# jibanCat/gp_dla_detection

Measured on AMD Instinct MI355X. Metric: sample log-likelihoods/sec (n~1500,k=20), higher is better.
Workload: dtype f64; 1 GPU; BASELINE configs[1]: synthetic spectra, fused Voigt + low-rank log-evidence sweep, HBM-resident; spectra_per_gpu=1000, pixels=1500, k=20, dla_samples=10000, num_lines=3, parallelism=spectra sharded over 1 GPU(s), RCCL all-gather of the 15-column posterior table

## Files before the change

### gp_dla_detection_amd/_lib.py

```python
from __future__ import annotations

import ctypes as C
import os
import subprocess

_HERE = os.path.dirname(os.path.abspath(__file__))
CSRC = os.path.join(_HERE, "csrc")
DEFAULT_LIB_PATH = os.path.join(CSRC, "libgpdla.so")


def lib_path() -> str:
    return os.environ.get("GPDLA_LIB_PATH") or DEFAULT_LIB_PATH

HIPCC_FLAGS = ["--offload-arch=gfx950", "-O3", "-ffp-contract=off", "-fPIC", "-shared",
               "-std=c++17", "-no-hip-rt", "-Wno-inline-asm"]

LEGACY_LIB_PATH = os.path.join(CSRC, "libgpdla_legacy.so")

_dp = C.POINTER(C.c_double)
_i64p = C.POINTER(C.c_int64)
_i32p = C.POINTER(C.c_int32)
_u8p = C.POINTER(C.c_uint8)
_u32p = C.POINTER(C.c_uint32)
_f32p = C.POINTER(C.c_float)
# ... 251 lines not shown
    ("gpdla_model_spectra_validate", C.c_int, [C.POINTER(ModelSpectraRequest), C.c_int64, C.c_int64, C.c_int]),
    ("gpdla_batch_unmasked_counts", C.c_int, [C.c_void_p, C.c_void_p, _i64p]),
    ("gpdla_batch_model_spectra", C.c_int, [C.c_void_p, C.c_void_p, C.POINTER(ModelSpectraRequest),
                                            C.POINTER(ModelSpectra)]),
    ("gpdla_model_spectra_multi_validate", C.c_int, [C.POINTER(ModelSpectraMultiRequest), C.c_int64, C.c_int64, C.c_int,
                                                     C.c_int, C.c_int]),
    ("gpdla_batch_model_spectra_multi", C.c_int, [C.c_void_p, C.c_void_p, C.POINTER(ModelSpectraMultiRequest),
                                                  C.POINTER(ModelSpectraMulti)]),
    ("gpdla_debug_profiles_ms", C.c_int, [C.c_void_p, C.c_void_p, _dp]),
    ("gpdla_model_mean", C.c_int, [C.POINTER(Model), C.c_int64, _dp, _i64p, _dp, _dp, C.c_int, C.c_int, C.c_int,
                                   C.c_double, C.c_double, _dp, C.c_int]),
    ("gpdla_mock_validate", C.c_int, [C.POINTER(MockRequest), C.c_int64]),
    ("gpdla_batch_draw_mocks", C.c_int, [C.c_void_p, C.c_void_p, C.POINTER(MockRequest), C.POINTER(MockSpectra)]),
    ("gpdla_samples_kde", C.c_int, [C.c_int64, _dp, C.c_int64, _dp, C.c_double, _dp, _dp, C.c_int]),
    ("gpdla_samples_fit_prior", C.c_int, [C.c_int64, _dp, C.c_double, C.c_double, C.c_double, C.c_double, C.c_double,
                                          C.c_double, C.c_double, C.c_double, C.POINTER(NhiPrior), C.c_int]),
    ("gpdla_samples_prior_eval", C.c_int, [C.POINTER(NhiPrior), C.c_int64, _dp, _dp, _dp, C.c_int]),
    ("gpdla_samples_halton", C.c_int, [C.c_int64, C.c_int64, C.c_int, _i32p, _dp, C.c_int]),
    ("gpdla_samples_draw", C.c_int, [C.POINTER(NhiPrior), C.c_int64, C.c_int64, _dp, C.c_int, C.c_double, C.c_double,
                                     C.POINTER(SampleDraw), C.c_int]),
    ("gpdla_preload_spectra", C.c_int, [C.c_int64, _i64p, _f32p, _f32p, _f32p, _i32p, _dp, _u8p, C.POINTER(PreloadConfig),
                                        _i64p, _dp, _dp, _dp, _u8p, _dp, C.c_int]),
    ("gpdla_stats_parameter_summaries", C.c_int, [C.c_int64, C.c_int64, _dp, C.c_int64, _u32p, _dp, _dp, _dp, _dp,
                                                  C.POINTER(SummaryRequest), C.POINTER(ParameterSummaries), C.c_int]),
    ("gpdla_batch_parameter_summaries", C.c_int, [C.c_void_p, C.c_void_p, C.c_int, C.c_int, _i64p, C.c_int64,
                                                  C.POINTER(SummaryRequest), C.POINTER(ParameterSummaries)]),
    ("gpdla_debug_last_summaries_ms", C.c_double, []),
    ("gpdla_refine_validate", C.c_int, [C.POINTER(RefineRequest), C.POINTER(NhiPrior), C.c_int64, _dp, _dp]),
    ("gpdla_context_set_refine_points", C.c_int, [C.c_void_p, C.c_int64, _dp, _dp]),
    ("gpdla_batch_refine", C.c_int, [C.c_void_p, C.c_void_p, _i64p, C.c_int64, C.POINTER(RefineRequest),
                                     C.POINTER(NhiPrior)]),
    ("gpdla_batch_download_refined", C.c_int, [C.c_void_p, C.c_void_p, _i64p, C.c_int64, C.POINTER(RefinedResults)]),
    ("gpdla_batch_refined_summaries", C.c_int, [C.c_void_p, C.c_void_p, _i64p, C.c_int64, C.POINTER(SummaryRequest),
                                                C.POINTER(ParameterSummaries)]),
    ("gpdla_batch_refined_posteriors", C.c_int, [C.c_void_p, C.c_void_p, _i64p, C.c_int64, C.POINTER(RefinedPosteriors)]),
    ("gpdla_debug_last_refine_ms", C.c_double, []),
    ("gpdla_fixed_absorbers_validate", C.c_int, [C.c_int64, _i64p, _dp, _dp, C.c_double]),
    ("gpdla_batch_set_fixed_absorbers", C.c_int, [C.c_void_p, C.c_void_p, _i64p, _dp, _dp, C.c_double, C.c_int32]),
    ("gpdla_batch_clear_fixed_absorbers", C.c_int, [C.c_void_p, C.c_void_p]),
    ("gpdla_debug_conditioned_rows", C.c_int, [C.c_void_p, C.c_void_p, C.c_int32, C.c_int64, _dp, _dp, C.c_int64, _i64p]),
    ("gpdla_stats_posterior_maps", C.c_int, [C.c_int64, C.c_int64, _dp, C.c_int64, _u32p, _dp, _dp, _dp, _dp, _dp, _dp, _dp, _dp,
                                             _dp, C.POINTER(PosteriorMapsRequest), C.POINTER(PosteriorMaps), C.c_int]),
    ("gpdla_batch_posterior_maps", C.c_int, [C.c_void_p, C.c_void_p, C.c_int, C.c_int, _i64p, C.c_int64, _dp, _dp, _dp, _dp,
                                             _dp, C.POINTER(PosteriorMapsRequest), C.POINTER(PosteriorMaps)]),
    ("gpdla_batch_refined_posterior_maps", C.c_int, [C.c_void_p, C.c_void_p, _i64p, C.c_int64, _dp, _dp, _dp, _dp, _dp,
                                                     C.POINTER(PosteriorMapsRequest), C.POINTER(PosteriorMaps)]),
    ("gpdla_posterior_maps_rows_per_launch", C.c_int64, [C.c_int, C.c_int, C.c_int]),
    ("gpdla_debug_last_maps_ms", C.c_double, [C.c_int]),
    ("gpdla_debug_last_maps_launches", C.c_int64, []),
    ("gpdla_debug_near_poly", C.c_int, [C.c_int, C.c_double, _dp, _dp]),
    ("gpdla_debug_prepared_rows", C.c_int, [C.c_void_p, C.c_void_p, C.c_int, C.c_int64, _dp, C.c_int64, _i64p]),
    ("gpdla_debug_philox4x32_10", None, [_u32p, _u32p, _u32p]),
    ("gpdla_debug_throw", C.c_int, [C.c_int]),
]

_lib = None


def host_sources() -> list:
    import re
    unit = os.path.join(CSRC, "gpdla.hip")
    with open(unit) as f:
        names = re.findall(r'^#include "(host_\w+\.hpp)"', f.read(), flags=re.M)
    return [unit] + [os.path.join(CSRC, n) for n in names]


def _build(out: str, extra_flags, force: bool, verbose: bool) -> str:
    import glob
    srcs = (host_sources() + glob.glob(os.path.join(CSRC, "*.hip")) + glob.glob(os.path.join(CSRC, "*.hpp"))
            + glob.glob(os.path.join(_HERE, "..", "include", "*.h")))
    if not force and os.path.exists(out):
        if all(os.path.getmtime(out) >= os.path.getmtime(s) for s in srcs):
            return out
    cmd = ["hipcc", *HIPCC_FLAGS, *extra_flags, os.path.join(CSRC, "gpdla.hip"), "-o", out]
    res = subprocess.run(cmd, capture_output=True, text=True)
    if verbose or res.returncode:
        print(res.stdout, res.stderr)
    if res.returncode:
        raise RuntimeError(f"hipcc failed building {os.path.basename(out)}:\n" + res.stderr)
    return out


def build(force: bool = False, verbose: bool = False) -> str:
    return _build(DEFAULT_LIB_PATH, [], force, verbose)


def build_legacy(force: bool = False, verbose: bool = False) -> str:
    return _build(LEGACY_LIB_PATH, ["-DGPDLA_WITH_LEGACY"], force, verbose)


def _preload_hip_runtime():
    candidates = []
    try:
        import torch
        candidates.append(os.path.join(os.path.dirname(torch.__file__), "lib", "libamdhip64.so"))
    except Exception:
        pass
    candidates += ["/opt/rocm/lib/libamdhip64.so", "libamdhip64.so"]
    last = None
    for path in candidates:
        if os.path.isabs(path) and not os.path.exists(path):
            continue
        try:
            return C.CDLL(path, mode=C.RTLD_GLOBAL)
        except OSError as e:
            last = e
# ... 26 lines not shown
```

### gp_dla_detection_amd/csrc/host_refine.hpp

```cpp
#pragma once

static_assert(GPDLA_REFINE_MAX_LEVELS == gpdla::kRefineMaxLevels, "gpdla.h and sweep_kernels.hpp disagree");

namespace {

thread_local double t_refine_ms = -1.0;

int validate_refine_request(const gpdla_refine_request *rq, const gpdla_nhi_prior *prior) {
  if (!rq) return fail(GPDLA_ERR_INVALID_ARGUMENT, "null refine request");
  if (rq->levels < 1 || rq->levels > GPDLA_REFINE_MAX_LEVELS)
    return fail(GPDLA_ERR_INVALID_ARGUMENT, "levels = %d outside [1, %d]", rq->levels, GPDLA_REFINE_MAX_LEVELS);
  if (!(rq->delta > 0.0) || !std::isfinite(rq->delta)) return fail(GPDLA_ERR_INVALID_ARGUMENT, "delta = %g must be finite and > 0", rq->delta);
  if (!(rq->pad >= 0.0) || !std::isfinite(rq->pad)) return fail(GPDLA_ERR_INVALID_ARGUMENT, "pad = %g must be finite and >= 0", rq->pad);
  return prior ? check_prior(prior) : GPDLA_OK;
}

int validate_refine_points(int64_t n, const double *u, const double *v) {
  if (n < 1 || n > (1LL << 30)) return fail(GPDLA_ERR_INVALID_ARGUMENT, "num_points = %lld outside [1, 2^30]", (long long)n);
  if (!u || !v) return fail(GPDLA_ERR_INVALID_ARGUMENT, "null u / v");
  for (int64_t j = 0; j < n; ++j) {
    if (!(u[j] >= 0.0 && u[j] < 1.0)) return fail(GPDLA_ERR_INVALID_ARGUMENT, "u[%lld] = %g is not inside [0, 1)", (long long)j, u[j]);
    if (!(v[j] >= 0.0 && v[j] < 1.0)) return fail(GPDLA_ERR_INVALID_ARGUMENT, "v[%lld] = %g is not inside [0, 1)", (long long)j, v[j]);
  }
  return GPDLA_OK;
}

size_t refine_layout(RefineBuffers *rf, char *base, size_t nq, size_t Sr) {
  size_t at = 0;
  auto take = [&](auto *&p, size_t count) {
    using T = std::remove_reference_t<decltype(*p)>;
    if (base) p = reinterpret_cast<T *>(base + at);
    at += (std::max<size_t>(count * sizeof(T), 8) + 255) & ~(size_t)255;
  };
  take(rf->box, nq * kRefineBoxStride);
  take(rf->rmeta, nq);
  take(rf->ell, nq * Sr);
  take(rf->lam, nq * Sr);
  take(rf->ll_scratch, nq);
  take(rf->terms, nq * kRefineTerms * 2);
  take(rf->scal, nq * kRefineScalars);
  take(rf->status, nq);
  take(rf->rows, nq);
  return at;
}

int refine_reserve(gpdla_batch *b, int64_t Sr) {
  if (!b->rf) b->rf = new RefineBuffers();
  RefineBuffers *rf = b->rf;
  if (!rf->ev_rows) HIP_TRY(hipEventCreateWithFlags(&rf->ev_rows, hipEventDisableTiming));
  const size_t need = refine_layout(rf, nullptr, (size_t)b->nq, (size_t)Sr);
  if (!rf->arena || rf->cap_bytes < need) {
    dev_free(rf->arena);
    rf->arena = nullptr;
    rf->cap_bytes = 0;
    void *p = nullptr;
    if (hipMalloc(&p, need) != hipSuccess) return fail(GPDLA_ERR_HIP, "hipMalloc of %zu bytes for the refine tables failed", need);
    rf->arena = p;
    rf->cap_bytes = need;
  }
  refine_layout(rf, static_cast<char *>(rf->arena), (size_t)b->nq, (size_t)Sr);
  rf->nq = b->nq;
  rf->Sr = Sr;
  return GPDLA_OK;
}

int launch_boxed_sweep(gpdla_context *c, gpdla_batch *b, RecordClass cls, int64_t count, const BoxedSweepArgs &args) {
  const bool three = args.num_lines == 3;
  if (cls == kRecSlim20)
    return launch_sweep_kernel(c, three ? &k_sweep_slim_boxed<3> : &k_sweep_slim_boxed<0>, kSweepWaves * 64,
                               (size_t)kSlimLdsDoubles * sizeof(double), kSweepWaves * kSamplesPerWave, count, args);
  const size_t lds = std::max(sweep_split_slim_lds_doubles(false), kExpTab + kSplitEpilogueDoubles) * sizeof(double);
  if (lds > 160 * 1024) return fail(GPDLA_ERR_UNSUPPORTED, "split sweep needs %zu B of LDS", lds);
  return launch_sweep_kernel(c, three ? &k_sweep_split_slim<3, 0, BoxedSweepArgs> : &k_sweep_split_slim<0, 0, BoxedSweepArgs>, 512, lds,
                             2 * kSamplesPerWave, count, args);
}

int check_refinable(gpdla_context *c, gpdla_batch *b) {
  int rc = check_batch_pair(c, b);
  if (rc) return rc;
  if (b->md) return fail(GPDLA_ERR_UNSUPPORTED, "the refine pass serves single-DLA batches only");
  if (c->cfg.contraction_precision == 1) return fail(GPDLA_ERR_UNSUPPORTED, "the refine pass is fp64 only (contraction_precision = 1)");
  if (b->k > 40) return fail(GPDLA_ERR_UNSUPPORTED, "k = %d: the refine pass serves k <= 40", b->k);
  return GPDLA_OK;
}

}

extern "C" {

int gpdla_refine_validate(const gpdla_refine_request *request, const gpdla_nhi_prior *prior, int64_t num_points,
                          const double *u, const double *v) try {
  int rc = validate_refine_request(request, prior);
  if (rc) return rc;
  return (num_points || u || v) ? validate_refine_points(num_points, u, v) : GPDLA_OK;
} GPDLA_NO_THROW

int gpdla_context_set_refine_points(gpdla_context *c, int64_t num_points, const double *u, const double *v) try {
  if (!c) return fail(GPDLA_ERR_INVALID_ARGUMENT, "null context");
  int rc = validate_refine_points(num_points, u, v);
  if (rc) return rc;
  HIP_TRY(hipSetDevice(c->device_id));
  HIP_TRY(hipStreamSynchronize(c->stream));
  dev_free(c->d_ru);
  dev_free(c->d_rv);
  dev_free(c->d_rperm);
  c->d_ru = c->d_rv = nullptr;
  c->d_rperm = nullptr;
  c->Sr = 0;
  const size_t n = (size_t)num_points;
  std::vector<int32_t> perm(n);
  std::iota(perm.begin(), perm.end(), 0);
  std::stable_sort(perm.begin(), perm.end(), [&](int32_t x, int32_t y) { return u[x] < u[y]; });
  if ((rc = upload(&c->d_ru, u, n, c->stream)) || (rc = upload(&c->d_rv, v, n, c->stream)) ||
      (rc = upload(&c->d_rperm, perm.data(), n, c->stream)))
    return rc;
  HIP_TRY(hipStreamSynchronize(c->stream));
  c->h_ru.assign(u, u + n);
  c->h_rv.assign(v, v + n);
  c->Sr = num_points;
  ++c->refine_points_gen;
  return GPDLA_OK;
} GPDLA_NO_THROW

// ... 206 lines not shown
    const int64_t q = selection ? selection[s] : s;
    const double *bx = box.data() + (size_t)q * kRefineBoxStride + 4 * (rf->levels - 1);
    z_lo[(size_t)s] = bx[0];
    z_hi[(size_t)s] = bx[1];
    n_lo[(size_t)s] = bx[2];
    n_hi[(size_t)s] = bx[3];
    row_start[(size_t)s] = q * Sr;
  }
  return run_parameter_summaries(nsel, Sr, rf->lam, row_start, nullptr, none, z_lo.data(), z_hi.data(), c->h_ru.data(),
                                 c->h_rv.data(), *request, *outputs, st, n_lo.data(), n_hi.data());
} GPDLA_NO_THROW

int gpdla_batch_refined_posteriors(gpdla_context *c, gpdla_batch *b, const int64_t *selection, int64_t num_selected,
                                   gpdla_refined_posteriors *out) try {
  int rc = check_refinable(c, b);
  if (rc) return rc;
  if (!out) return fail(GPDLA_ERR_INVALID_ARGUMENT, "null outputs");
  if ((rc = check_selection(b->nq, selection, num_selected))) return rc;
  RefineBuffers *rf = b->rf;
  if (!rf || rf->levels < 1 || rf->nq != b->nq) return fail(GPDLA_ERR_INVALID_ARGUMENT, "the batch has not been refined");
  const int64_t n = num_selected;
  if (n == 0) return GPDLA_OK;
  HIP_TRY(hipSetDevice(c->device_id));
  std::vector<int64_t> sel((size_t)n);
  for (int64_t s = 0; s < n; ++s) sel[(size_t)s] = selection ? selection[s] : s;
  std::vector<double> post((size_t)n * 4);
  Staging up(c->stream);
  HIP_TRY(hipStreamWaitEvent(c->stream, b->ev_done, 0));
  RefinedPosteriorArgs a{};
  int64_t *d_sel;
  if ((rc = up.put(&d_sel, sel.data(), (size_t)n)) || (rc = up.tmp.alloc(&a.post, (size_t)n * 4)) ||
      (rc = up.tmp.alloc(&a.refined, (size_t)n)))
    return rc;
  a.n = n;
  a.sel = d_sel;
  a.summary = b->d_summary;
  a.scal = rf->scal;
  a.status = rf->status;
  hipLaunchKernelGGL(k_refined_posteriors, dim3((unsigned)((n + 255) / 256)), dim3(256), 0, c->stream, a);
  HIP_TRY(hipGetLastError());
  if ((rc = up.fetch(post.data(), a.post, post.size())) || (rc = up.fetch(out->refined, a.refined, (size_t)n))) return rc;
  HIP_TRY(hipStreamSynchronize(c->stream));
  for (int64_t s = 0; s < n; ++s) {
    const double *p = post.data() + 4 * s;
    if (out->model_posteriors_refined) std::memcpy(out->model_posteriors_refined + 2 * s, p, 2 * sizeof(double));
    if (out->p_no_dlas_refined) out->p_no_dlas_refined[s] = p[2];
    if (out->p_dlas_refined) out->p_dlas_refined[s] = p[3];
  }
  return GPDLA_OK;
} GPDLA_NO_THROW

double gpdla_debug_last_refine_ms(void) { return t_refine_ms; }

}
```

### gp_dla_detection_amd/csrc/host_sweep.hpp

```cpp
#pragma once

namespace {

template <typename Args>
int launch_sweep_kernel(gpdla_context *c, void (*kernel)(Args), int threads, size_t lds, int samples_per_block,
                        int64_t num_quasars, Args args) {
  HIP_TRY(hipFuncSetAttribute(reinterpret_cast<const void *>(kernel), hipFuncAttributeMaxDynamicSharedMemorySize, (int)lds));
  args.blocks_per_quasar = (int32_t)((args.S + 1 + samples_per_block - 1) / samples_per_block);
  const int64_t nblocks = 8 * ((num_quasars + 7) / 8) * (int64_t)args.blocks_per_quasar;
  if (nblocks > 2147483647LL) return fail(GPDLA_ERR_UNSUPPORTED, "batch too large for one launch");
  hipLaunchKernelGGL(kernel, dim3((unsigned)nblocks), dim3(threads), lds, c->stream, args);
  HIP_TRY(hipGetLastError());
  return GPDLA_OK;
}

template <class F>
int dispatch_nd(int mode, F &&f) {
  switch (mode == 0 ? 1 : mode) {
    case 1: return f(std::integral_constant<int, 1>{});
    case 2: return f(std::integral_constant<int, 2>{});
    case 3: return f(std::integral_constant<int, 3>{});
    case 4: return f(std::integral_constant<int, 4>{});
    default: return fail(GPDLA_ERR_UNSUPPORTED, "max_dlas = %d > 4", mode);
  }
// ... 75 lines not shown
  pa.num_forest_lines = c->cfg.num_forest_lines;
  pa.prev_tau_0 = c->cfg.prev_tau_0;
  pa.prev_beta = c->cfg.prev_beta;
  hipLaunchKernelGGL(k_prepare, dim3((unsigned)b->nq), dim3(256), 0, st, pa);
  HIP_TRY(hipGetLastError());
  return GPDLA_OK;
}

enum RecordClass { kRecExpanded = 0, kRecSlim20 = 1, kRecSlim40 = 2 };
int64_t record_class_doubles(RecordClass rc, int ntiles, bool f32_tiles) {
  return rc == kRecSlim20 ? kSlimRec : rc == kRecSlim40 ? kS40Rec : record_doubles(ntiles, f32_tiles ? 1 : 0);
}
int launch_build_records(gpdla_context *c, gpdla_batch *b, int64_t g0, int64_t g1, bool f32_tiles, RecordClass cls) {
  const bool slim = cls != kRecExpanded;
  BuildRecordsArgs ba;
  ba.meta = b->d_meta;
  ba.pix = b->d_pix;
  ba.Mi = b->d_Mi;
  ba.lam_pad = b->d_lam;
  ba.records = b->d_records;
  ba.k = b->k;
  ba.tiles_w = b->tiles_w;
  ba.ntiles = b->ntiles;
  ba.blocks_per_quasar = slim ? 4 : 16;
  ba.f32_tiles = f32_tiles ? 1 : 0;
  ba.order = b->d_order + g0;
  const unsigned grid = (unsigned)((g1 - g0) * ba.blocks_per_quasar);
  if (cls == kRecSlim20)
    hipLaunchKernelGGL(k_build_slim_records, dim3(grid), dim3(256), 0, c->stream, ba);
  else if (cls == kRecSlim40)
    hipLaunchKernelGGL(k_build_slim40_records, dim3(grid), dim3(256), 0, c->stream, ba);
  else
    hipLaunchKernelGGL(k_build_records, dim3(grid), dim3(256), 0, c->stream, ba);
  HIP_TRY(hipGetLastError());
  return GPDLA_OK;
}

RecordClass legacy_record_class(int k, RecordClass product);
template <int KMAX>
int legacy_sweep(gpdla_context *c, gpdla_batch *b, const SweepArgs &args);
template <class Args>
int legacy_sweep_multi(gpdla_context *c, gpdla_batch *b, const Args &args);

bool is_conditioned(const gpdla_batch *b) { return b->fx && b->fx->on; }
int check_conditionable(const gpdla_context *c, const gpdla_batch *b);
int launch_condition_rows(gpdla_context *c, gpdla_batch *b);
int launch_condition_mask(gpdla_context *c, gpdla_batch *b, const int32_t *rows, int64_t count, const int32_t *status,
                          const double *box, const double *su, int64_t S, double *table);

int launch_sweep(gpdla_context *c, gpdla_batch *b, RecordClass cls, bool f32, const SweepArgs &args) {
  const bool three = args.num_lines == 3;
  if (b->k <= 20) {
    if (cls == kRecSlim20)
      return launch_sweep_kernel(c, three ? &k_sweep_slim<3> : &k_sweep_slim<0>, kSweepWaves * 64,
                                 (size_t)kSlimLdsDoubles * sizeof(double), kSweepWaves * kSamplesPerWave, b->nq, args);
    if (!f32) return legacy_sweep<20>(c, b, args);
    return three ? launch_sweep_expanded<float, 8, 14, 1, 8, 13, 3>(c, b, args) : launch_sweep_expanded<float, 8, 14, 1, 4, 13, 0>(c, b, args);
  }
  if (cls == kRecSlim40) {
    const size_t lds = std::max(sweep_split_slim_lds_doubles(false), kExpTab + kSplitEpilogueDoubles) * sizeof(double);
    if (lds > 160 * 1024) return fail(GPDLA_ERR_UNSUPPORTED, "split sweep needs %zu B of LDS", lds);
    return launch_sweep_kernel(c, three ? &k_sweep_split_slim<3, 0, SweepArgs> : &k_sweep_split_slim<0, 0, SweepArgs>, 512, lds,
                               2 * kSamplesPerWave, args.nq, args);
  }
  if (!f32) return legacy_sweep<40>(c, b, args);
  return three ? launch_sweep_expanded<float, 4, 56, 1, 4, 52, 3>(c, b, args) : launch_sweep_expanded<float, 4, 56, 1, 4, 52, 0>(c, b, args);
}

}

extern "C" {

int gpdla_batch_process(gpdla_context *c, gpdla_batch *b) try {
  if (!c || !b || b->ctx != c) return fail(GPDLA_ERR_INVALID_ARGUMENT, "null/mismatched context or batch");
  if (b->S != c->S || b->k != c->model.k)
    return fail(GPDLA_ERR_INVALID_ARGUMENT, "model/samples changed after the batch was uploaded");
  if (b->md) return fail(GPDLA_ERR_INVALID_ARGUMENT, "multi-DLA batch: use gpdla_batch_process_multi");
  if (b->k > 40) return fail(GPDLA_ERR_UNSUPPORTED, "k = %d needs %d B tiles (max 56)", b->k, b->ntiles);
  HIP_TRY(hipSetDevice(c->device_id));
  hipStream_t st = c->stream;
  const bool f32 = c->cfg.contraction_precision == 1;
  const RecordClass cls = legacy_record_class(b->k, f32 ? kRecExpanded : b->k <= 20 ? kRecSlim20 : kRecSlim40);
  const bool conditioned = is_conditioned(b);
  int rc = conditioned ? check_conditionable(c, b) : GPDLA_OK;
  if (rc || (rc = plan_records(c, b, record_class_doubles(cls, b->ntiles, false), false))) return rc;
  if ((rc = launch_prepare(c, b, conditioned && b->fx->meanflux))) return rc;
  if (conditioned && (rc = launch_condition_rows(c, b))) return rc;

  HIP_TRY(hipMemsetAsync(b->d_sample_ll, 0xFF, (size_t)b->nq * b->S * sizeof(double), st));
  HIP_TRY(hipMemsetAsync(b->d_ll_no, 0xFF, (size_t)b->nq * sizeof(double), st));

  SweepArgs sa;
  sa.meta = b->d_meta;
  sa.records = b->d_records;
  sa.lam_pad = b->d_lam;
  sa.offset_samples = c->d_offset;
  sa.nhi_samples = c->d_nhi;
  sa.perm = c->d_perm;
  sa.pix = b->d_pix;
  sa.S = b->S;
  sa.k = b->k;
  sa.tiles_w = b->tiles_w;
  sa.ntiles = b->ntiles;
  sa.num_lines = c->cfg.num_lines;
  sa.sample_ll = b->d_sample_ll;
  sa.ll_no_dla = b->d_ll_no;
  sa.blocks_per_quasar = 0;
  if ((rc = begin_timing(c, st))) return rc;
// ... 204 lines not shown
```

### gp_dla_detection_amd/csrc/sweep_slim_body.hpp

```cpp
template <int LINES>
__global__ __launch_bounds__(512) void GPDLA_SWEEP_SLIM_KERNEL(GPDLA_SWEEP_SLIM_ARGS a) {
  static_assert(LINES == 3 || LINES == 0, "three lines at compile time, or a run-time count");
  extern __shared__ double smem[];
  constexpr int WAVES = kSweepWaves, CH = kSlimCH;
  const int64_t xj = blockIdx.x >> 3;
  const int64_t pos = 8 * (xj / a.blocks_per_quasar) + (blockIdx.x & 7);
  const int bq = (int)(xj % a.blocks_per_quasar);
  if (pos >= a.nq) return;
  const int64_t q = a.order[pos];
  const QuasarMeta m = a.meta[q];
  if (m.status != 0) return;
  const int tid = threadIdx.x, wave = tid >> 6, lane = tid & 63;
  const int s = lane & 15, jj = lane >> 4;

  double *ring = smem;
  double *blocks = ring + kSlimRingD;
  double *land = blocks + 2 * kSlimBlock + wave * kSlimLand;
  const double *exp_pad = ring + 32;

  const int64_t slot0 = (int64_t)bq * (WAVES * kSamplesPerWave) + wave * kSamplesPerWave;
  const int64_t slot = slot0 + s;
  const bool is_sample = slot < a.S;
  const bool is_null = !is_sample;
  const int32_t sample = a.perm[is_sample ? slot : a.S - 1];
  const double z_dla = m.min_z_dla + (m.max_z_dla - m.min_z_dla) * a.offset_samples[sample];
  double nhi = a.nhi_samples[sample];
  if constexpr (std::is_same_v<GPDLA_SWEEP_SLIM_ARGS, BoxedSweepArgs> && LINES >= 0) {
    const double *box = sweep_box(a, q);
    nhi = exp10(box[2] + (box[3] - box[2]) * nhi);
  }
  [[maybe_unused]] double mult_r[3];
  [[maybe_unused]] const double opz = 1 + z_dla, inv_opz = 1.0 / opz;
  [[maybe_unused]] const int L = LINES > 0 ? LINES : a.num_lines;
  if constexpr (LINES == 3) {
#pragma unroll
    for (int j = 0; j < 3; ++j) mult_r[j] = g_lines.c / (g_lines.wavelength_cm[j] * (1 + z_dla)) / 1e8;
  }
  if (tid < kExpTab) ring[tid * kRing2 + 32] = exp2((double)tid * (1.0 / kExpTab));
  double *my_ring = ring + (size_t)(wave * kSamplesPerWave + s) * kRing2 + jj;
  const double *lam = a.lam_pad + m.lam_off;
  const int n_pad = m.n_u + 6;
  const double nscale64 = -nhi * g_lines.inv_sqrt2pi_sigma * kInvSqrtPi * kExpScale;
  const double *rec_base = a.records + m.rec_off * (int64_t)kSlimRec;
  const int nchunks = (m.steps + CH - 1) / CH;

  const int wave_s = __builtin_amdgcn_readfirstlane(wave);
  const uint32_t raw_lds = __builtin_amdgcn_readfirstlane(lds_address(blocks + kSlimTileBuf));
  auto issue_chunk = [&](int c) {
    glds_chunk<CH * kSlimRec / 128, WAVES>(rec_base + (size_t)c * CH * kSlimRec,
                                           raw_lds + (uint32_t)(c & 1) * (uint32_t)(kSlimBlock * 8), wave_s, lane);
  };
  const double *land_src = rec_base + (size_t)wave_s * kSlimRec;
  const int src_rows = 4 * kSlimExtras + 16 * jj + 2 * (s & 7);
  const int src_x = kSlimExtras * (lane >> 1) + 4 + 2 * (lane & 1);
  auto issue_private = [&](int c) {
    const double *rec = land_src + (size_t)c * CH * kSlimRec;
    glds16(rec + src_rows, land);
    if (lane < 8) glds16(rec + src_x, land + 4 * 32);
  };
  const double *row = land + 32 * jj + s;
  const double *bc = land + 4 * 32 + 4 * jj;
  const double *a8 = s < 8 ? row : bc + (slim_pair_i(8, s) - 16);
  const double *b8 = s < 8 ? row + 8 : bc + (slim_pair_j(8, s) - 16);
  struct Operands {
    double mc, o[2], p8;
  };
  auto expand_load = [&](int t0, int t1, Operands &x) {
    x.mc = row[0];
#pragma unroll
    for (int t = t0; t < t1; ++t) {
      if (t == 8) {
        x.o[t - t0] = a8[0];
        x.p8 = b8[0];
      } else {
        x.o[t - t0] = t == 0 ? x.mc : t < 8 ? row[t] : bc[t - 9];
      }
    }
  };
  auto expand_store = [&](double *dst, int t0, int t1, const Operands &x) {
#pragma unroll
    for (int t = t0; t < t1; ++t) dst[t * 64] = (t == 8 ? x.p8 : x.mc) * x.o[t - t0];
  };
  double *const xd0 = blocks + (size_t)wave_s * kSlimStepTiles + lane;
  const double *const tb0 = blocks + lane;
  const double *const mb0 = blocks + kSlimTileBuf + kSlimExtras * jj;
  const double *const ub0 = blocks + kSlimTileBuf + 4 * kSlimExtras + lane;
  auto pinned = [](const double *p) {
    uint32_t v = lds_address(p);
    asm volatile("" : "+v"(v));
    return (double *)(__attribute__((address_space(3))) double *)(uintptr_t)v;
  };

  issue_private(0);
  issue_chunk(0);

  const double c_light = g_lines.c, inv_s = g_lines.inv_sqrt2_sigma;
  [[maybe_unused]] double ms_r[3];
  if constexpr (LINES == 3) {
#pragma unroll
    for (int j = 0; j < 3; ++j) ms_r[j] = mult_r[j] * inv_s;
  }
  const double cs = c_light * inv_s;
  auto optical_sum = [&](double lamP) -> double {
    if constexpr (LINES == 3) {
      bool near;
      double total = wing_sum3(lamP, ms_r[0], ms_r[1], ms_r[2], cs, &near);
      if (__builtin_expect(__any(near), 0)) total = total_near<3>(lamP, mult_r[0], mult_r[1], mult_r[2], nullptr, 3);
      return total;
    } else {
      bool near;
      double total = wing_sum_runtime(lamP * inv_opz, cs, L, &near);
      if (__builtin_expect(__any(near), 0)) total = total_near_at(lamP, opz, L);
      return total;
    }
  };

  __syncthreads();
  for (int c3 = 0; c3 < 3; ++c3) {
    const double lam0 = lam[min(4 * c3 + jj, n_pad - 1)];
    const double tot = optical_sum(lam0);
    const ExpState es0 = exp_ring_begin_scaled(nscale64 * tot, exp_pad);
    const double v = exp_table_end_scaled(es0);
    my_ring[4 * c3] = v;
    my_ring[4 * c3 + 16] = v;
  }

  d4 acc[14];
#pragma unroll
  for (int c = 0; c < 14; ++c) acc[c] = d4{0, 0, 0, 0};
  double quad_sum = 0.0, dprod = 1.0;
  double xw[kXW] = {0.0, 0.0}, xu[kXU] = {0.0, 0.0, 0.0, 0.0};
  int dexp = 0;
  const double tap0 = g_lines.taps[0], tap1 = g_lines.taps[1], tap2 = g_lines.taps[2], tap3 = g_lines.taps[3];

  glds_wait();
  {
    const double mc = row[0];
    for (int t = 0; t < kSlimTilesW; ++t)
      xd0[t * 64] = (t == 8 ? b8[0] : mc) * (t == 8 ? a8[0] : t == 0 ? mc : t < 8 ? row[t] : bc[t - 9]);
  }
  __builtin_amdgcn_s_waitcnt(0xC07F);
  if (nchunks > 1) issue_private(1);
  glds_wait();
  __syncthreads();

  for (int c = 0; c < nchunks; ++c) {
    __builtin_amdgcn_s_waitcnt(0x0070);
    if (c + 1 < nchunks) issue_chunk(c + 1);
    const int par = (c & 1) * kSlimBlock;
    const double *tbuf = pinned(tb0 + par);
    const double *mine0 = pinned(mb0 + par);
    const double *ubuf = pinned(ub0 + par);
    double *xdst = pinned(xd0 + (kSlimBlock - par));
    double lam_next = 0.0;
    double n0 = 0.0, n1 = 0.0, n2 = 0.0, n3 = 0.0, n4 = 0.0, n5 = 0.0, n6 = 0.0;
    double2 n01 = {0.0, 0.0}, n23 = {0.0, 0.0};
#pragma unroll
    for (int tt = 0; tt < CH; ++tt) {
      const int rn = c * CH + tt;
      constexpr int kXS = 7;
      constexpr int kT0[7] = {0, 2, 4, 6, 8, 10, 12}, kT1[7] = {2, 4, 6, 8, 10, 12, 13};
      if (tt == kXS && c + 2 < nchunks) issue_private(c + 2);
      if (rn < m.steps) {
        const double *tl = tbuf + (size_t)tt * kSlimStepTiles;
        const double *mine = mine0 + (size_t)tt * kSlimRec;
        const int slot_p = (4 * tt) & 15;
        const int slot_w = (slot_p + 12) & 15;
        if (tt > 0) __builtin_amdgcn_s_waitcnt(0xC07F);
        const double lamP = tt == 0 ? mine[10] : lam_next;
        double g0 = n0, g1 = n1, g2 = n2, g3 = n3, g4 = n4, g5 = n5, g6 = n6;
        double2 p01 = n01, p23 = n23;
        if (tt == 0) {
          const double *g = my_ring + slot_p;
          g0 = g[0], g1 = g[1], g2 = g[2], g3 = g[3], g4 = g[4], g5 = g[5], g6 = g[6];
          p01 = *reinterpret_cast<const double2 *>(mine);
          p23 = *reinterpret_cast<const double2 *>(mine + 2);
        }
        const double py = p01.x, pmu = p01.y, pom = p23.x, pnu = p23.y;
        __builtin_amdgcn_sched_barrier(0);
        [[maybe_unused]] WingFront wf;
        [[maybe_unused]] bool near = false;
        if constexpr (LINES == 3) {
          if (tt == 0) {
            wf = wing3_front(lamP, ms_r[0], ms_r[1], ms_r[2], cs, &near);
            __builtin_amdgcn_sched_barrier(0);
          }
        }
        double absorb = fma(g6, tap0, g0 * tap0);
        {
          double ab2 = fma(g5, tap1, g1 * tap1);
          absorb = fma(g2, tap2, absorb);
          ab2 = fma(g4, tap2, ab2);
          absorb = fma(g3, tap3, absorb) + ab2;
        }
        if (is_null) absorb = 1.0;
        const double a2 = absorb * absorb;
        const double d = fma(pom, a2, pnu);
        double inv_d;
        double total;
        if constexpr (LINES == 3) {
          if (tt > 0) wf = wing3_front(lamP, ms_r[0], ms_r[1], ms_r[2], cs, &near);
          total = wing3_back_rcp4(wf, d, &inv_d);
#ifndef SLIM_EXP_NONEAR
          if (__builtin_expect(__any(near), 0)) total = total_near<3>(lamP, mult_r[0], mult_r[1], mult_r[2], nullptr, 3);
#endif
        } else {
          total = optical_sum(lamP);
          inv_d = fast_rcp(d);
        }
        const ExpState es = exp_ring_begin_scaled(nscale64 * total, exp_pad);
        __builtin_amdgcn_sched_barrier(0);
        double bop[14];
#pragma unroll
        for (int cc = 0; cc < kSlimTilesW; ++cc) bop[cc] = tl[cc * 64];
        bop[13] = ubuf[(size_t)tt * kSlimRec];
        __builtin_amdgcn_sched_barrier(0);
        const double pser = exp_series_scaled(es);
        const double r = fma(-absorb, pmu, py);
        const double w = a2 * inv_d;
        const double ri = r * inv_d;
        const double u = absorb * ri;
        quad_sum = fma(r, ri, quad_sum);
        dprod *= d;
        if (tt & 1) {
          dexp += __builtin_amdgcn_frexp_exp(dprod);
          dprod = __builtin_amdgcn_frexp_mant(dprod);
        }
        __builtin_amdgcn_sched_barrier(0);
        const double raw = exp_finish_scaled(es, pser);
        my_ring[slot_w] = raw;
        my_ring[slot_w + 16] = raw;
        Operands x;
        if (tt < kXS) expand_load(kT0[tt < kXS ? tt : 0], kT1[tt < kXS ? tt : 0], x);
        if (tt + 1 < CH) lam_next = mine[kSlimRec + 10];
        __builtin_amdgcn_sched_barrier(0);
        constexpr int kSplit = 11;
        const double2 xp = *reinterpret_cast<const double2 *>(mine + 8);
        const double2 u01 = *reinterpret_cast<const double2 *>(mine + 4);
        const double2 u23 = *reinterpret_cast<const double2 *>(mine + 6);
#pragma unroll
        for (int cc = 0; cc < kSplit; ++cc)
          acc[cc] = __builtin_amdgcn_mfma_f64_16x16x4f64(cc < kSlimTilesW ? w : u, bop[cc], acc[cc], 0, 0, 0);
        if (tt < kXS) expand_store(xdst, kT0[tt < kXS ? tt : 0], kT1[tt < kXS ? tt : 0], x);
        if (tt + 1 < CH) {
          __builtin_amdgcn_sched_barrier(0);
          const double *g = my_ring + ((4 * (tt + 1)) & 15);
          n0 = g[0], n1 = g[1], n2 = g[2], n3 = g[3], n4 = g[4], n5 = g[5], n6 = g[6];
          n01 = *reinterpret_cast<const double2 *>(mine + kSlimRec);
          n23 = *reinterpret_cast<const double2 *>(mine + kSlimRec + 2);
          __builtin_amdgcn_sched_barrier(0);
        }
#pragma unroll
        for (int cc = kSplit; cc < 14; ++cc)
          acc[cc] = __builtin_amdgcn_mfma_f64_16x16x4f64(cc < kSlimTilesW ? w : u, bop[cc], acc[cc], 0, 0, 0);
        xw[0] = fma(w, xp.x, xw[0]);
        xw[1] = fma(w, xp.y, xw[1]);
        xu[0] = fma(u, u01.x, xu[0]);
        xu[1] = fma(u, u01.y, xu[1]);
        xu[2] = fma(u, u23.x, xu[2]);
        xu[3] = fma(u, u23.y, xu[3]);
      }
    }
    glds_wait();
    __syncthreads();
  }

  double logd_sum = log(dprod) + (double)dexp * 0.6931471805599453;
  quad_sum += __shfl_xor(quad_sum, 16);
  quad_sum += __shfl_xor(quad_sum, 32);
  logd_sum += __shfl_xor(logd_sum, 16);
  logd_sum += __shfl_xor(logd_sum, 32);
#pragma unroll
  for (int x = 0; x < kXW; ++x) {
    xw[x] += __shfl_xor(xw[x], 16);
    xw[x] += __shfl_xor(xw[x], 32);
  }
#pragma unroll
  for (int x = 0; x < kXU; ++x) {
    xu[x] += __shfl_xor(xu[x], 16);
    xu[x] += __shfl_xor(xu[x], 32);
  }

  using ES = EpilogueShape<13, 1>;
  double *Eg = smem + (size_t)wave * ES::SPP * ES::stride(16);
#pragma unroll
  for (int p = 0; p < ES::PASSES; ++p) {
    int sigma;
    bool writer;
    const double ll = slim_factor_pass(acc, xw, xu, p, Eg, lane, a.k, quad_sum, logd_sum, m.n_kept, &sigma, &writer);
    const int64_t slot_s = slot0 + sigma;
    const int32_t sample_s = __shfl(sample, sigma + 16 * jj);
    if (writer) {
      if (slot_s < a.S) a.sample_ll[(int64_t)q * a.S + sample_s] = ll + m.ll_bias;
      else if (slot_s == a.S) a.ll_no_dla[q] = ll + m.ll_bias;
    }
  }
}
```

### gp_dla_detection_amd/csrc/sweep_slim_kernel.hpp

```cpp
#pragma once
#include <type_traits>

#include "sweep_kernels.hpp"

namespace gpdla {

constexpr int kSlimExtras = 12;
constexpr int kSlimRec = 4 * kSlimExtras + 64;
constexpr int kSlimCH = 8;
constexpr int kSlimTilesW = 13;
constexpr int kSlimStepTiles = kSlimTilesW * 64;
constexpr int kSlimRingD = kSweepWaves * kSamplesPerWave * kRing2;
constexpr int kSlimTileBuf = kSlimCH * kSlimStepTiles;
constexpr int kSlimRawBuf = kSlimCH * kSlimRec;
constexpr int kSlimLand = 4 * 32 + 4 * 4;
constexpr int kSlimBlock = kSlimTileBuf + kSlimRawBuf;
constexpr int kSlimLdsDoubles = kSlimRingD + 2 * kSlimBlock + kSweepWaves * kSlimLand;
static_assert((kSlimBlock * 8) % 512 == 0, "both parities reachable with ds_read2st64 offsets");
static_assert(kSlimLdsDoubles * 8 == 160 * 1024, "the slim sweep uses the whole LDS of a CU");
static_assert((kSlimCH * kSlimRec) % 128 == 0, "a raw chunk is a whole number of KiB");

__host__ __device__ constexpr int slim_pair_i(int tile, int col) {
  if (tile < 8) {
    const int b = (col + tile) & 15;
    return col > b ? col : b;
  }
  if (tile == 8) {
    if (col < 8) return col + 8;
    const int l = col - 8;
    return l < 1 ? 16 : l < 3 ? 17 : l < 6 ? 18 : 19;
  }
  return 16 + (tile - 9);
}
__host__ __device__ constexpr int slim_pair_j(int tile, int col) {
  if (tile < 8) {
    const int b = (col + tile) & 15;
    return col > b ? b : col;
  }
  if (tile == 8) {
    if (col < 8) return col;
    const int l = col - 8;
    return 16 + (l < 1 ? 0 : l < 3 ? l - 1 : l < 6 ? l - 3 : l - 6);
  }
  return col;
}
__host__ __device__ constexpr int slim_pos(int tile, int col) {
  return slim_pair_i(tile, col) * (slim_pair_i(tile, col) + 1) / 2 + slim_pair_j(tile, col);
}

__global__ __launch_bounds__(256) void k_build_slim_records(BuildRecordsArgs a) {
  const int q = a.order[blockIdx.x / a.blocks_per_quasar];
  const int bq = blockIdx.x % a.blocks_per_quasar;
  const QuasarMeta m = a.meta[q];
  const int k = a.k;
  const int n_pad = m.n_u + 6;
  double *out = a.records + m.rec_off * (int64_t)kSlimRec;
  const int64_t total = (int64_t)(m.steps + 1) * kSlimRec;
  for (int64_t e = (int64_t)bq * 256 + threadIdx.x; e < total; e += (int64_t)a.blocks_per_quasar * 256) {
    const int step = (int)(e / kSlimRec), r = (int)(e - (int64_t)step * kSlimRec);
    double v = 0.0;
    if (r < 4 * kSlimExtras) {
      const int jj = r / kSlimExtras, f = r - jj * kSlimExtras;
      const int64_t row = m.pix_off + 4 * (int64_t)step + jj;
      if (f < 4) {
        const PixelRow px = a.pix[row];
        v = f == 0 ? px.y : f == 1 ? px.mu : f == 2 ? px.omega2 : px.nu;
      } else if (f < 8) {
        if (kXUColumn + (f - 4) < k) v = a.Mi[row * k + kXUColumn + (f - 4)];
      } else if (f < 10) {
        if (k == 20) v = a.Mi[row * k + 19] * a.Mi[row * k + 18 + (f - 8)];
      } else if (f == 10) {
        int P = 4 * (step + 3) + jj;
        if (P > n_pad - 1) P = n_pad - 1;
// ... 106 lines not shown
```

### include/gpdla.h

```cpp
#ifndef GPDLA_H
#define GPDLA_H

#include <stdint.h>

#ifdef __cplusplus
extern "C" {
#endif

typedef enum {
  GPDLA_OK = 0,
  GPDLA_ERR_INVALID_ARGUMENT = -1,
  GPDLA_ERR_NO_DEVICE = -2,
  GPDLA_ERR_HIP = -3,
  GPDLA_ERR_NOT_POSITIVE_DEFINITE = -4,
  GPDLA_ERR_UNSUPPORTED = -5,
  GPDLA_ERR_HOST = -6
} gpdla_status;

#define GPDLA_MAX_K 40
#define GPDLA_ABI_VERSION 6

int gpdla_abi_version(void);
const char *gpdla_last_error(void);

// ... 149 lines not shown
                              const gpdla_spectra *spectra, const uint32_t *base_sample_inds,
                              const gpdla_config *config, gpdla_results_multi *results,
                              int device_id);

int gpdla_process_cells_multi(const gpdla_model *model, const gpdla_samples *samples,
                              const gpdla_spectra_cells *spectra, const uint32_t *base_sample_inds,
                              const gpdla_config *config, gpdla_results_multi *results,
                              int device_id);

int gpdla_batch_process_multi(gpdla_context *ctx, gpdla_batch *batch,
                              const uint32_t *base_sample_inds);
int gpdla_batch_download_multi(gpdla_context *ctx, gpdla_batch *batch, gpdla_results_multi *results);

#define GPDLA_SUMMARY_COLS_MULTI(md) (14 + 4 * (md) + 3 * (md) * (md))
int gpdla_batch_summary_multi_device_ptr(gpdla_batch *batch, double **table, int64_t *num_quasars,
                                         int32_t *num_cols);
int gpdla_batch_samples_multi_device_ptr(gpdla_batch *batch, double **sample_ll_dla,
                                         double **sample_ll_lls, uint32_t **base_sample_inds);

typedef struct gpdla_training gpdla_training;
int gpdla_training_create(int device_id, int64_t num_quasars, int64_t num_pixels,
                          const double *centered_rest_fluxes, const double *lya_1pzs,
                          const double *rest_noise_variances, gpdla_training **out);
int gpdla_training_objective(gpdla_training *t, const double *x, int k, double *f, double *g);
int gpdla_training_set_lyseries(gpdla_training *t, int num_forest_lines, const double *all_transition_wavelengths,
                                const double *all_oscillator_strengths);
void gpdla_training_destroy(gpdla_training *t);

typedef struct {
  double min_lambda, dlambda;
  int64_t num_rest_pixels;
  double lya_wavelength;
  double max_noise_variance;
  double prev_tau_0, prev_beta;
  int32_t num_forest_lines;
} gpdla_learn_config;

int gpdla_training_create_from_spectra(int device_id, const gpdla_spectra *spectra, const gpdla_learn_config *config,
                                       gpdla_training **out);
int gpdla_training_column_stats(gpdla_training *t, double *mu, double *std, int64_t *count);
int gpdla_training_pca_covariance(gpdla_training *t, int complete_rows, double *cov, double *count,
                                  int64_t *rows_used);
int gpdla_training_download(gpdla_training *t, double *flux, double *lya, double *noise);

int gpdla_debug_near_poly(int line, double x, double *value_out, double *y_out);

int gpdla_debug_prepared_rows(gpdla_context *ctx, gpdla_batch *batch, int multi, int64_t quasar,
                              double *rows_out, int64_t capacity_rows, int64_t *num_rows_out);

void gpdla_debug_philox4x32_10(const uint32_t ctr[4], const uint32_t key[2], uint32_t out[4]);

int gpdla_debug_throw(int kind);

#define GPDLA_STATS_MAX_BINS 64
#define GPDLA_STATS_MAX_REQUESTS 4
#define GPDLA_STATS_KEPT_CAPACITY 8
typedef struct {
  int32_t quantity;
  int32_t num_bins;
  const double *edges;
  double z_lo, z_hi, lnhi_lo, lnhi_hi;
  int32_t histogram, moment, lowzcut;
  double p_thresh_sample, p_switch;
} gpdla_bin_request;
typedef struct {
  double *pois, *mean, *var;
  int32_t *kept_count;
  int32_t *kept_bin;
  double *kept_p;
} gpdla_bin_output;
int gpdla_stats_bin_posteriors(int64_t num_spectra, int64_t num_samples, const double *sample_log_likelihoods,
                               int64_t row_stride, const double *shift, const double *p_dla, const double *z_min,
                               const double *z_max, const double *upper_z, const double *offset_samples,
                               const double *log_nhi_samples, int num_requests, const gpdla_bin_request *requests,
                               gpdla_bin_output *outputs, int device_id);
int gpdla_stats_poisson_binomial_cf(int64_t num_segments, const int64_t *offsets, const double *p, double *logsum,
                                    double *argsum, int device_id);

int gpdla_stats_bin_posteriors_boxed(int64_t num_rows, int64_t num_points, const double *sample_log_posteriors,
                                     int64_t row_stride, const double *p_dla, const double *boxes, const double *upper_z,
                                     const double *u, const double *v, int num_requests,
                                     const gpdla_bin_request *requests, gpdla_bin_output *outputs, double *shift,
                                     int device_id);
void gpdla_debug_time_bin_kernels(int on);
double gpdla_debug_last_bin_ms(void);

#define GPDLA_BOOTSTRAP_MAX_COLUMNS 256
int gpdla_stats_sightline_snrs(int64_t num_sightlines, const int64_t *offsets, const double *wavelengths,
                               const double *flux, const double *noise_variance, const double *max_z_dlas,
                               const double *normalizers, double *snrs, int device_id);
int gpdla_stats_path_lengths(int64_t num_sightlines, const double *min_z_dlas, const double *max_z_dlas,
                             int num_bins, const double *edges, int lowzcut, double proximity_zone, double omega_m,
                             double *dX, int device_id);
int gpdla_stats_bootstrap_sums(int64_t num_rows, int num_columns, const double *V, const int32_t *stratum,
                               uint64_t seed, int64_t first_replicate, int64_t num_replicates, double *sums,
                               int device_id);

#define GPDLA_SPECTRA_MAX_ABSORBERS 8
#define GPDLA_SPECTRA_MAP 1
#define GPDLA_SPECTRA_MOMENTS 2
#define GPDLA_SPECTRA_CONTINUUM 4
#define GPDLA_SPECTRA_WEIGHTS_NONE 0
#define GPDLA_SPECTRA_WEIGHTS_RESIDENT 1
#define GPDLA_SPECTRA_WEIGHTS_HOST 2
typedef struct {
  int64_t num_selected;
// ... 246 lines not shown
```

Before: 68.88 million evals/s.

## Halve slim sweep block to four waves so two blocks share each CU

The slim k<=20 sweep kernel goes from a 512-thread block that filled all 160 KiB of LDS to a 4-wave block with half the chunk depth and 80 KiB of LDS, with launch bounds asking for two blocks per CU. Two independent blocks can then overlap each other's barriers and load phases. The raw-record copy now has each wave copy one record with per-lane 16-byte global-to-LDS loads, and the ring reads for the next chunk are hoisted into the last step of the previous chunk. Risks are smaller per-block prefetch depth, a tighter register budget from the occupancy hint, and a new debug occupancy query.

Result: faster. 69.90 million evals/s (median of 6 runs) (+1.5%).

```diff
diff --git a/gp_dla_detection_amd/_lib.py b/gp_dla_detection_amd/_lib.py
--- a/gp_dla_detection_amd/_lib.py
+++ b/gp_dla_detection_amd/_lib.py
@@ -327,6 +327,7 @@
     ("gpdla_debug_prepared_rows", C.c_int, [C.c_void_p, C.c_void_p, C.c_int, C.c_int64, _dp, C.c_int64, _i64p]),
     ("gpdla_debug_philox4x32_10", None, [_u32p, _u32p, _u32p]),
     ("gpdla_debug_throw", C.c_int, [C.c_int]),
+    ("gpdla_debug_slim_sweep_blocks_per_cu", C.c_int, [C.c_int, C.POINTER(C.c_int)]),
 ]
 
 _lib = None
diff --git a/gp_dla_detection_amd/csrc/host_refine.hpp b/gp_dla_detection_amd/csrc/host_refine.hpp
--- a/gp_dla_detection_amd/csrc/host_refine.hpp
+++ b/gp_dla_detection_amd/csrc/host_refine.hpp
@@ -67,8 +67,8 @@
 int launch_boxed_sweep(gpdla_context *c, gpdla_batch *b, RecordClass cls, int64_t count, const BoxedSweepArgs &args) {
   const bool three = args.num_lines == 3;
   if (cls == kRecSlim20)
-    return launch_sweep_kernel(c, three ? &k_sweep_slim_boxed<3> : &k_sweep_slim_boxed<0>, kSweepWaves * 64,
-                               (size_t)kSlimLdsDoubles * sizeof(double), kSweepWaves * kSamplesPerWave, count, args);
+    return launch_sweep_kernel(c, three ? &k_sweep_slim_boxed<3> : &k_sweep_slim_boxed<0>, kSlimWaves * 64,
+                               (size_t)kSlimLdsDoubles * sizeof(double), kSlimWaves * kSamplesPerWave, count, args);
   const size_t lds = std::max(sweep_split_slim_lds_doubles(false), kExpTab + kSplitEpilogueDoubles) * sizeof(double);
   if (lds > 160 * 1024) return fail(GPDLA_ERR_UNSUPPORTED, "split sweep needs %zu B of LDS", lds);
   return launch_sweep_kernel(c, three ? &k_sweep_split_slim<3, 0, BoxedSweepArgs> : &k_sweep_split_slim<0, 0, BoxedSweepArgs>, 512, lds,
@@ -381,4 +381,16 @@
 
 double gpdla_debug_last_refine_ms(void) { return t_refine_ms; }
 
-}
+int gpdla_debug_slim_sweep_blocks_per_cu(int kernel, int *blocks_out) try {
+  if (!blocks_out || kernel < 0 || kernel > 3)
+    return fail(GPDLA_ERR_INVALID_ARGUMENT, "gpdla_debug_slim_sweep_blocks_per_cu: kernel %d", kernel);
+  const void *const f[4] = {reinterpret_cast<const void *>(&k_sweep_slim<3>), reinterpret_cast<const void *>(&k_sweep_slim<0>),
+                            reinterpret_cast<const void *>(&k_sweep_slim_boxed<3>),
+                            reinterpret_cast<const void *>(&k_sweep_slim_boxed<0>)};
+  const size_t lds = (size_t)kSlimLdsDoubles * sizeof(double);
+  HIP_TRY(hipFuncSetAttribute(f[kernel], hipFuncAttributeMaxDynamicSharedMemorySize, (int)lds));
+  HIP_TRY(hipOccupancyMaxActiveBlocksPerMultiprocessor(blocks_out, f[kernel], kSlimWaves * 64, lds));
+  return GPDLA_OK;
+} GPDLA_NO_THROW
+
+}
diff --git a/gp_dla_detection_amd/csrc/host_sweep.hpp b/gp_dla_detection_amd/csrc/host_sweep.hpp
--- a/gp_dla_detection_amd/csrc/host_sweep.hpp
+++ b/gp_dla_detection_amd/csrc/host_sweep.hpp
@@ -151,8 +151,8 @@
   const bool three = args.num_lines == 3;
   if (b->k <= 20) {
     if (cls == kRecSlim20)
-      return launch_sweep_kernel(c, three ? &k_sweep_slim<3> : &k_sweep_slim<0>, kSweepWaves * 64,
-                                 (size_t)kSlimLdsDoubles * sizeof(double), kSweepWaves * kSamplesPerWave, b->nq, args);
+      return launch_sweep_kernel(c, three ? &k_sweep_slim<3> : &k_sweep_slim<0>, kSlimWaves * 64,
+                                 (size_t)kSlimLdsDoubles * sizeof(double), kSlimWaves * kSamplesPerWave, b->nq, args);
     if (!f32) return legacy_sweep<20>(c, b, args);
     return three ? launch_sweep_expanded<float, 8, 14, 1, 8, 13, 3>(c, b, args) : launch_sweep_expanded<float, 8, 14, 1, 4, 13, 0>(c, b, args);
   }
diff --git a/gp_dla_detection_amd/csrc/sweep_slim_body.hpp b/gp_dla_detection_amd/csrc/sweep_slim_body.hpp
--- a/gp_dla_detection_amd/csrc/sweep_slim_body.hpp
+++ b/gp_dla_detection_amd/csrc/sweep_slim_body.hpp
@@ -1,8 +1,8 @@
 template <int LINES>
-__global__ __launch_bounds__(512) void GPDLA_SWEEP_SLIM_KERNEL(GPDLA_SWEEP_SLIM_ARGS a) {
+__global__ __launch_bounds__(kSlimWaves * 64, 2) void GPDLA_SWEEP_SLIM_KERNEL(GPDLA_SWEEP_SLIM_ARGS a) {
   static_assert(LINES == 3 || LINES == 0, "three lines at compile time, or a run-time count");
   extern __shared__ double smem[];
-  constexpr int WAVES = kSweepWaves, CH = kSlimCH;
+  constexpr int WAVES = kSlimWaves, CH = kSlimSweepCH;
   const int64_t xj = blockIdx.x >> 3;
   const int64_t pos = 8 * (xj / a.blocks_per_quasar) + (blockIdx.x & 7);
   const int bq = (int)(xj % a.blocks_per_quasar);
@@ -14,8 +14,8 @@
   const int s = lane & 15, jj = lane >> 4;
 
   double *ring = smem;
-  double *blocks = ring + kSlimRingD;
-  double *land = blocks + 2 * kSlimBlock + wave * kSlimLand;
+  double *blocks = ring + kSlimSweepRingD;
+  double *land = blocks + 2 * kSlimSweepBlock + wave * kSlimLand;
   const double *exp_pad = ring + 32;
 
   const int64_t slot0 = (int64_t)bq * (WAVES * kSamplesPerWave) + wave * kSamplesPerWave;
@@ -45,10 +45,10 @@
   const int nchunks = (m.steps + CH - 1) / CH;
 
   const int wave_s = __builtin_amdgcn_readfirstlane(wave);
-  const uint32_t raw_lds = __builtin_amdgcn_readfirstlane(lds_address(blocks + kSlimTileBuf));
+  double *const raw_mine = blocks + kSlimSweepTileBuf + wave_s * kSlimRec;
+  const double *const raw_src = rec_base + (size_t)wave_s * kSlimRec + 2 * lane;
   auto issue_chunk = [&](int c) {
-    glds_chunk<CH * kSlimRec / 128, WAVES>(rec_base + (size_t)c * CH * kSlimRec,
-                                           raw_lds + (uint32_t)(c & 1) * (uint32_t)(kSlimBlock * 8), wave_s, lane);
+    if (lane < kSlimRec / 2) glds16(raw_src + (size_t)c * CH * kSlimRec, raw_mine + (c & 1) * kSlimSweepBlock);
   };
   const double *land_src = rec_base + (size_t)wave_s * kSlimRec;
   const int src_rows = 4 * kSlimExtras + 16 * jj + 2 * (s & 7);
@@ -63,7 +63,7 @@
   const double *a8 = s < 8 ? row : bc + (slim_pair_i(8, s) - 16);
   const double *b8 = s < 8 ? row + 8 : bc + (slim_pair_j(8, s) - 16);
   struct Operands {
-    double mc, o[2], p8;
+    double mc, o[5], p8;
   };
   auto expand_load = [&](int t0, int t1, Operands &x) {
     x.mc = row[0];
@@ -83,8 +83,8 @@
   };
   double *const xd0 = blocks + (size_t)wave_s * kSlimStepTiles + lane;
   const double *const tb0 = blocks + lane;
-  const double *const mb0 = blocks + kSlimTileBuf + kSlimExtras * jj;
-  const double *const ub0 = blocks + kSlimTileBuf + 4 * kSlimExtras + lane;
+  const double *const mb0 = blocks + kSlimSweepTileBuf + kSlimExtras * jj;
+  const double *const ub0 = blocks + kSlimSweepTileBuf + 4 * kSlimExtras + lane;
   auto pinned = [](const double *p) {
     uint32_t v = lds_address(p);
     asm volatile("" : "+v"(v));
@@ -144,22 +144,22 @@
   glds_wait();
   __syncthreads();
 
+  double n0 = my_ring[0], n1 = my_ring[1], n2 = my_ring[2], n3 = my_ring[3], n4 = my_ring[4], n5 = my_ring[5], n6 = my_ring[6];
   for (int c = 0; c < nchunks; ++c) {
     __builtin_amdgcn_s_waitcnt(0x0070);
     if (c + 1 < nchunks) issue_chunk(c + 1);
-    const int par = (c & 1) * kSlimBlock;
+    const int par = (c & 1) * kSlimSweepBlock;
     const double *tbuf = pinned(tb0 + par);
     const double *mine0 = pinned(mb0 + par);
     const double *ubuf = pinned(ub0 + par);
-    double *xdst = pinned(xd0 + (kSlimBlock - par));
+    double *xdst = pinned(xd0 + (kSlimSweepBlock - par));
     double lam_next = 0.0;
-    double n0 = 0.0, n1 = 0.0, n2 = 0.0, n3 = 0.0, n4 = 0.0, n5 = 0.0, n6 = 0.0;
     double2 n01 = {0.0, 0.0}, n23 = {0.0, 0.0};
 #pragma unroll
     for (int tt = 0; tt < CH; ++tt) {
       const int rn = c * CH + tt;
-      constexpr int kXS = 7;
-      constexpr int kT0[7] = {0, 2, 4, 6, 8, 10, 12}, kT1[7] = {2, 4, 6, 8, 10, 12, 13};
+      constexpr int kXS = 3;
+      constexpr int kT0[3] = {0, 5, 9}, kT1[3] = {5, 9, 13};
       if (tt == kXS && c + 2 < nchunks) issue_private(c + 2);
       if (rn < m.steps) {
         const double *tl = tbuf + (size_t)tt * kSlimStepTiles;
@@ -171,8 +171,6 @@
         double g0 = n0, g1 = n1, g2 = n2, g3 = n3, g4 = n4, g5 = n5, g6 = n6;
         double2 p01 = n01, p23 = n23;
         if (tt == 0) {
-          const double *g = my_ring + slot_p;
-          g0 = g[0], g1 = g[1], g2 = g[2], g3 = g[3], g4 = g[4], g5 = g[5], g6 = g[6];
           p01 = *reinterpret_cast<const double2 *>(mine);
           p23 = *reinterpret_cast<const double2 *>(mine + 2);
         }
@@ -249,6 +247,11 @@
           n01 = *reinterpret_cast<const double2 *>(mine + kSlimRec);
           n23 = *reinterpret_cast<const double2 *>(mine + kSlimRec + 2);
           __builtin_amdgcn_sched_barrier(0);
+        } else {
+          __builtin_amdgcn_sched_barrier(0);
+          const double *g = my_ring;
+          n0 = g[0], n1 = g[1], n2 = g[2], n3 = g[3], n4 = g[4], n5 = g[5], n6 = g[6];
+          __builtin_amdgcn_sched_barrier(0);
         }
 #pragma unroll
         for (int cc = kSplit; cc < 14; ++cc)
diff --git a/gp_dla_detection_amd/csrc/sweep_slim_kernel.hpp b/gp_dla_detection_amd/csrc/sweep_slim_kernel.hpp
--- a/gp_dla_detection_amd/csrc/sweep_slim_kernel.hpp
+++ b/gp_dla_detection_amd/csrc/sweep_slim_kernel.hpp
@@ -10,15 +10,26 @@
 constexpr int kSlimCH = 8;
 constexpr int kSlimTilesW = 13;
 constexpr int kSlimStepTiles = kSlimTilesW * 64;
-constexpr int kSlimRingD = kSweepWaves * kSamplesPerWave * kRing2;
 constexpr int kSlimTileBuf = kSlimCH * kSlimStepTiles;
 constexpr int kSlimRawBuf = kSlimCH * kSlimRec;
 constexpr int kSlimLand = 4 * 32 + 4 * 4;
 constexpr int kSlimBlock = kSlimTileBuf + kSlimRawBuf;
-constexpr int kSlimLdsDoubles = kSlimRingD + 2 * kSlimBlock + kSweepWaves * kSlimLand;
 static_assert((kSlimBlock * 8) % 512 == 0, "both parities reachable with ds_read2st64 offsets");
-static_assert(kSlimLdsDoubles * 8 == 160 * 1024, "the slim sweep uses the whole LDS of a CU");
 static_assert((kSlimCH * kSlimRec) % 128 == 0, "a raw chunk is a whole number of KiB");
+constexpr int kSlimWaves = 4;
+constexpr int kSlimSweepCH = 4;
+constexpr int kSlimSweepRingD = kSlimWaves * kSamplesPerWave * kRing2;
+constexpr int kSlimSweepTileBuf = kSlimSweepCH * kSlimStepTiles;
+constexpr int kSlimSweepBlock = kSlimSweepTileBuf + kSlimSweepCH * kSlimRec;
+constexpr int kSlimLdsDoubles = kSlimSweepRingD + 2 * kSlimSweepBlock + kSlimWaves * kSlimLand;
+static_assert(kSlimSweepCH == kSlimWaves, "wave w expands, and copies, K-step w of the next chunk");
+static_assert((kSlimSweepBlock * 8) % 512 == 0, "both parities reachable with ds_read2st64 offsets");
+static_assert(kSlimLdsDoubles * 8 == 80 * 1024, "two blocks of the slim sweep fill the LDS of a CU exactly");
+static_assert(kSlimWaves * kSamplesPerWave == kExpTab, "the exp table has one ring row's pad slot per entry");
+static_assert((kSlimSweepCH * 4) % 16 == 0, "the ring slots of a K-step depend on its place in the chunk alone");
+static_assert(kSlimRec % 2 == 0 && kSlimRec / 2 <= 64, "one wave copies one record, 16 bytes per lane");
+static_assert(kSlimWaves * EpilogueShape<13, 1>::SPP * EpilogueShape<13, 1>::stride(16) <= kSlimLdsDoubles,
+              "the epilogue's rows fit the block's LDS");
 
 __host__ __device__ constexpr int slim_pair_i(int tile, int col) {
   if (tile < 8) {
diff --git a/include/gpdla.h b/include/gpdla.h
--- a/include/gpdla.h
+++ b/include/gpdla.h
@@ -225,6 +225,8 @@
 
 int gpdla_debug_throw(int kind);
 
+int gpdla_debug_slim_sweep_blocks_per_cu(int kernel, int *blocks_out);
+
 #define GPDLA_STATS_MAX_BINS 64
 #define GPDLA_STATS_MAX_REQUESTS 4
 #define GPDLA_STATS_KEPT_CAPACITY 8
```
